# astojanov/Clover

Measured on AMD Instinct MI355X. Metric: int4 GEMV (CloverMatrix4::mvm) effective GB/s, algorithmic operand bytes / time, higher is better.
Workload: dtype int4; 1 GPU; CloverMatrix4::mvm 65536x65536 int4 (65536x65536 per GPU; preset c3: BASELINE configs[2] per GPU), x and result CloverVector4, STOCHASTIC_ROUNDING_DISABLED, bit-exact reference order; rows_per_gpu=65536, cols=65536, parallelism=row-shard x1, settle_launches=168

## Files before the change

clover_amd/csrc/matrix4.hip:

```cpp
#include "rng_device.h"

#include <stdlib.h>
#include <string.h>


#define MVM_CHUNK 65536u

template <int U, bool NT>
__device__ __forceinline__ void mvm_steps(const u32x4 *__restrict__ Ap, const u32x4 *xs, const float *cs, int q,
                                          uint32_t t0, float &a0, float &a1, float &a2, float &a3)
{
    u32x4 a[U];
#pragma unroll
    for (int u = 0; u < U; u++) a[u] = NT ? __builtin_nontemporal_load(&Ap[4 * (t0 + u) + q]) : Ap[4 * (t0 + u) + q];
#pragma unroll
    for (int u = 0; u < U; u++) {
        const u32x4 xv = xs[4 * (t0 + u) + q];
        const float c = cs[2 * (t0 + u) + (q >> 1)];
        a0 = __builtin_fmaf(c, (float)sdot8(a[u].x, xv.x, 0), a0);
        a1 = __builtin_fmaf(c, (float)sdot8(a[u].y, xv.y, 0), a1);
        a2 = __builtin_fmaf(c, (float)sdot8(a[u].z, xv.z, 0), a2);
        a3 = __builtin_fmaf(c, (float)sdot8(a[u].w, xv.w, 0), a3);
    }
}

template <int U, bool NT>
__device__ __forceinline__ void mvm_steps8(const u32x2 *__restrict__ Ap, const u32x2 *xs, const float *cs, int e, uint32_t t0, float &a0,
                                           float &a1)
{
    u32x2 a[U];
#pragma unroll
    for (int u = 0; u < U; u++) a[u] = NT ? __builtin_nontemporal_load(&Ap[8 * (t0 + u) + e]) : Ap[8 * (t0 + u) + e];
#pragma unroll
    for (int u = 0; u < U; u++) {
        const u32x2 xv = xs[8 * (t0 + u) + e];
        const float c = cs[2 * (t0 + u) + (e >> 2)];
        a0 = __builtin_fmaf(c, (float)sdot8(a[u].x, xv.x, 0), a0);
        a1 = __builtin_fmaf(c, (float)sdot8(a[u].y, xv.y, 0), a1);
    }
}

__device__ __forceinline__ int requantize_wave(float d, float noise, uint32_t *r_words, float *sr, float *scale)
{
    const int lane = threadIdx.x & 63;
    float m = wave_max(__builtin_fabsf(d));
    m = fix_zero_max(m);
    const float k = 7.0f / m;
    const int qv = quant1(d, k, noise);
    if (r_words) {
        uint32_t w = ((uint32_t)qv & 0xFu) << nib_shift(lane & 7);
        w |= __shfl_xor(w, 1);
        w |= __shfl_xor(w, 2);
        w |= __shfl_xor(w, 4);
        if ((lane & 7) == 0) r_words[lane >> 3] = w;
        if (lane == 0) *sr = m;
    }
    *scale = m;
    return qv;
}

struct MvmFuse {
    const uint32_t *qu;
    const float *su;
    float a;
    uint32_t *r2;
    float *sr2;
};

template <int U, bool NT, bool ST, bool FUSE, int L = 4>
__global__ __launch_bounds__(64 * L) void k_m4_mvm64(const uint8_t *__restrict__ A, const float *__restrict__ sA,
                                                  uint64_t cols, const uint8_t *__restrict__ x, const float *__restrict__ sx,
                                                  float *__restrict__ d_out, uint32_t *r, float *sr,
                                                  uint64_t *rng_state, uint64_t seq, const uint64_t *__restrict__ pow_rows, MvmFuse fuse)
{
    extern __shared__ __attribute__((aligned(16))) char smem[];
    u32x4 *xs = reinterpret_cast<u32x4 *>(smem);
    float *cs = reinterpret_cast<float *>(smem + MVM_CHUNK / 2);
    float *dsh = cs + MVM_CHUNK / 64;
    uint64_t *rbase = reinterpret_cast<uint64_t *>(dsh + 64);
    uint64_t *raw = rbase + 4;
    uint64_t *rbase2 = raw + 8, *raw2 = rbase2 + 4;
    if (ST) {
        const uint64_t a0 = rng_workgroup_begin(rng_state, seq, pow_rows, blockIdx.x, 1, (FUSE ? 4ull : 2ull) * gridDim.x, rbase);
        if (FUSE) {
            const uint64_t b2 = wave_pow_apply(pow_rows, a0, (uint64_t)gridDim.x + blockIdx.x, 1);
            if ((threadIdx.x & 63) == 0) rbase2[threadIdx.x >> 6] = b2;
        }
    }
    uint32_t fuse_w = 0;
    float fuse_s = 0.0f;
    if (FUSE && threadIdx.x < 64) {
        fuse_w = fuse.qu[blockIdx.x * 8 + (threadIdx.x >> 3)];
        fuse_s = fuse.su[blockIdx.x];
    }

    static_assert(L == 4 || (L == 8 && !ST), "the stochastic epilogue assumes 4 waves");
    constexpr int THREADS = 64 * L;
    const uint64_t rb = blockIdx.x;
    const int tid = threadIdx.x;
    const int q = tid & (L - 1);
    const int rho = tid / L;
    const uint64_t row = rb * 64 + rho;
    const u32x4 *Arow = reinterpret_cast<const u32x4 *>(A + row * (cols / 2));
    const float *sArow = sA + rb * (cols / 64);

    float a0 = 0.0f, a1 = 0.0f, a2 = 0.0f, a3 = 0.0f;

    for (uint64_t c0 = 0; c0 < cols; c0 += MVM_CHUNK) {
        const uint32_t cw = (uint32_t)((cols - c0) < MVM_CHUNK ? (cols - c0) : MVM_CHUNK);
        if (c0) __syncthreads();
        const u32x4 *xg = reinterpret_cast<const u32x4 *>(x + c0 / 2);
        {
            constexpr int NX = MVM_CHUNK / 32 / THREADS;
            constexpr int NC = MVM_CHUNK / 64 / THREADS;
            u32x4 xr[NX];
            float sa[NC], sv[NC];
            const uint32_t nx = cw / 32, nc = cw / 64;
#pragma unroll
            for (int k = 0; k < NX; k++) { const uint32_t i = tid + THREADS * k; xr[k] = xg[i < nx ? i : 0]; }
#pragma unroll
            for (int k = 0; k < NC; k++) {
                const uint32_t i = tid + THREADS * k, ii = i < nc ? i : 0;
                sa[k] = sArow[c0 / 64 + ii];
                sv[k] = sx[c0 / 64 + ii];
            }
#pragma unroll
            for (int k = 0; k < NX; k++) { const uint32_t i = tid + THREADS * k; if (i < nx) xs[i] = xr[k]; }
#pragma unroll
            for (int k = 0; k < NC; k++) { const uint32_t i = tid + THREADS * k; if (i < nc) cs[i] = (sa[k] * CLV_RCP49) * sv[k]; }
        }
        __syncthreads();

        const u32x4 *Ap = Arow + c0 / 32;
        const uint32_t npairs = cw / 128;
        uint32_t t = 0;
        if constexpr (L == 4) {
            for (; t + U <= npairs; t += U) mvm_steps<U, NT>(Ap, xs, cs, q, t, a0, a1, a2, a3);
            for (; t < npairs; t++) mvm_steps<1, NT>(Ap, xs, cs, q, t, a0, a1, a2, a3);
        } else {
            const u32x2 *Ap8 = reinterpret_cast<const u32x2 *>(Ap);
            const u32x2 *xs8 = reinterpret_cast<const u32x2 *>(xs);
            for (; t + U <= npairs; t += U) mvm_steps8<U, NT>(Ap8, xs8, cs, q, t, a0, a1);
            for (; t < npairs; t++) mvm_steps8<1, NT>(Ap8, xs8, cs, q, t, a0, a1);
        }
    }

    const float v0 = a0 + __shfl_xor(a0, 2);
    const float v1 = a1 + __shfl_xor(a1, 2);
    const float v2 = a2 + __shfl_xor(a2, 2);
    const float v3 = a3 + __shfl_xor(a3, 2);
    const float x0 = v0 + __shfl_xor(v0, 1);
    const float x1 = v1 + __shfl_xor(v1, 1);
    const float x2 = v2 + __shfl_xor(v2, 1);
    const float x3 = v3 + __shfl_xor(v3, 1);
    float dot = (x0 + x2) + (x1 + x3);
    if constexpr (L == 8) {
        const float u0 = a0 + __shfl_xor(a0, 4), u1 = a1 + __shfl_xor(a1, 4);
        const float y0 = u0 + __shfl_xor(u0, 2), y1 = u1 + __shfl_xor(u1, 2);
        const float z0 = y0 + __shfl_xor(y0, 1), z1 = y1 + __shfl_xor(y1, 1);
        dot = z0 + z1;
    }

    if (q == 0) {
        dsh[rho] = dot;
        if (d_out) d_out[row] = dot;
    }
    if (ST && tid < 4) {
        gen_blocks(rbase[tid], 1, raw, tid);
        if (FUSE) gen_blocks(rbase2[tid], 1, raw2, tid);
    }
    __syncthreads();
    if ((r || FUSE) && tid < 64) {
        float noise = 0.0f;
        if (ST) {
            const int grp = tid & 7, j = tid >> 3;
            noise = noise_of(reinterpret_cast<const uint32_t *>(raw + (size_t)(grp >> 2) * 4)[j], grp & 3);
        }
        float m;
        const int qv = requantize_wave(dsh[tid], noise, r ? r + rb * 8 : nullptr, r ? sr + rb : nullptr, &m);
        if (FUSE) {
            const float su7 = div7(fuse_s), sv7 = div7(m * fuse.a);
            const float val = __builtin_fmaf((float)qv, sv7, (float)unpack1(fuse_w, tid & 7) * su7);
            float noise2 = 0.0f;
            if (ST) {
                const int g = (tid & 7) ^ 1, j = tid >> 3;
                noise2 = noise_of(reinterpret_cast<const uint32_t *>(raw2 + (size_t)(g >> 2) * 4)[j], g & 3);
            }
            float m2;
            requantize_wave(val, noise2, fuse.r2 + rb * 8, fuse.sr2 + rb, &m2);
        }
    }
}

__global__ __launch_bounds__(256) void k_m4_quantize_strip(const float *__restrict__ A, uint64_t cols, uint32_t *__restrict__ q,
                                                           float *__restrict__ s, uint32_t strips_x, uint32_t tiles_x)
{
    __shared__ float sh[4][4];
    const uint32_t sj = blockIdx.x % strips_x;
    const uint64_t bi = blockIdx.x / strips_x;
    const int wave = threadIdx.x >> 6, lane = threadIdx.x & 63;
    const uint64_t col = (uint64_t)sj * 256 + 4 * lane;
    const bool live = col < cols;
    const uint64_t row0 = bi * 64 + wave * 16;

    f32x4 v[16];
    float m = 0.0f;
#pragma unroll
    for (int r = 0; r < 16; r++) {
        v[r] = live ? __builtin_nontemporal_load(reinterpret_cast<const f32x4 *>(A + (row0 + r) * cols + col)) : f32x4{0.0f, 0.0f, 0.0f, 0.0f};
        m = fmaxf(m, fmaxf(fmaxf(__builtin_fabsf(v[r].x), __builtin_fabsf(v[r].y)), fmaxf(__builtin_fabsf(v[r].z), __builtin_fabsf(v[r].w))));
    }
    m = row16_max(m);
    if ((lane & 15) == 0) sh[wave][lane >> 4] = m;
    __syncthreads();
    const int t = lane >> 4;
    m = fix_zero_max(fmaxf(fmaxf(sh[0][t], sh[1][t]), fmaxf(sh[2][t], sh[3][t])));
    const float k = 7.0f / m;
    if (wave == 0 && (lane & 15) == 0 && live) s[bi * tiles_x + sj * 4 + t] = m;
    const int odd = lane & 1;
#pragma unroll
    for (int r = 0; r < 16; r += 2) {
        const uint32_t h0 = quant_pack4(v[r], k), h1 = quant_pack4(v[r + 1], k);
        const uint32_t give = odd ? h0 : h1;
        const uint32_t recv = (uint32_t)__builtin_amdgcn_update_dpp(0, (int)give, 0xB1, 0xF, 0xF, false);
        const uint32_t word = odd ? (recv | (h1 << 16)) : (h0 | (recv << 16));
        if (live) __builtin_nontemporal_store(word, &q[((row0 + r + odd) * cols + (col & ~7ull)) / 8]);
    }
}

__global__ __launch_bounds__(256) void k_m4_gemm_simple(const uint8_t *__restrict__ A, const float *__restrict__ sA, uint64_t M,
                                                        uint64_t K, const uint8_t *__restrict__ B, const float *__restrict__ sB,
                                                        uint64_t N, float *__restrict__ C)
{
    const uint64_t j = (uint64_t)blockIdx.x * 16 + (threadIdx.x & 15);
    const uint64_t i = (uint64_t)blockIdx.y * 16 + (threadIdx.x >> 4);
    if (i >= M || j >= N) return;
    const uint64_t kb = K / 64;
    const u32x4 *a = reinterpret_cast<const u32x4 *>(A + i * (K / 2));
    const u32x4 *b = reinterpret_cast<const u32x4 *>(B + j * (K / 2));
    const float *sa = sA + (i >> 6) * kb;
    const float *sb = sB + (j >> 6) * kb;
    float acc = 0.0f;
    for (uint64_t blk = 0; blk < kb; blk++) {
        const int S = dot32(a[2 * blk], b[2 * blk]) + dot32(a[2 * blk + 1], b[2 * blk + 1]);
        const float c = (sa[blk] * CLV_RCP49) * sb[blk];
        acc = __builtin_fmaf(c, (float)S, acc);
    }
    C[i * N + j] = acc;
}

template <bool NT>
__global__ __launch_bounds__(256) void k_m4_restore(const uint32_t *__restrict__ q, const float *__restrict__ s, f32x4 *__restrict__ A,
                                                    uint64_t nquads, uint64_t cols)
{
    const uint64_t f0 = ((uint64_t)blockIdx.x * 4 + (threadIdx.x >> 6)) * 256;
    const int lane = threadIdx.x & 63;
    const uint64_t tiles_x = cols / 64;
    uint32_t wd[4];
    float sc[4];
#pragma unroll
    for (int j = 0; j < 4; j++) {
        const uint64_t f = f0 + 64 * j + lane, fc = f < nquads ? f : 0;
        const uint64_t e = fc * 4, row = e / cols, col = e - row * cols;
        wd[j] = q[fc >> 1];
        sc[j] = s[(row >> 6) * tiles_x + (col >> 6)];
    }
#pragma unroll
    for (int j = 0; j < 4; j++) {
        const uint64_t f = f0 + 64 * j + lane;
        const uint32_t hw = wd[j] >> (16 * (lane & 1));
        const float k = div7(sc[j]);
        f32x4 v;
        v.x = (float)(((int)(hw << 24)) >> 28) * k;
        v.y = (float)(((int)(hw << 28)) >> 28) * k;
        v.z = (float)(((int)(hw << 16)) >> 28) * k;
        v.w = (float)(((int)(hw << 20)) >> 28) * k;
        if (f < nquads) {
            if (NT) __builtin_nontemporal_store(v, &A[f]);
            else A[f] = v;
        }
    }
}

int clm4_quantize_stochastic(const float *A, uint64_t rows, uint64_t cols, int8_t *q, float *s, uint64_t *rng, hipStream_t st);
int clm4_gemm_mfma(const int8_t *A, const float *sA, uint64_t M, uint64_t K, const int8_t *B, const float *sB, uint64_t N, float *C, hipStream_t st);
int clm4_gemm_fp6(const int8_t *A, const float *sA, uint64_t M, uint64_t K, const int8_t *B, const float *sB, uint64_t N, float *C, hipStream_t st);

#define MVM_LDS_BYTES (MVM_CHUNK / 2 + (MVM_CHUNK / 64) * sizeof(float) + 64 * sizeof(float) + 256)

static int launch_mvm(const int8_t *A, const float *sA, uint64_t rows, uint64_t cols, const int8_t *x, const float *sx,
                      float *d, int8_t *r, float *sr, uint64_t *rng, hipStream_t st, const MvmFuse *fuse = nullptr)
{
    const size_t lds = MVM_LDS_BYTES;
    const dim3 grid((unsigned)(rows / 64)), block(256);
    RngTables T = {nullptr, nullptr, nullptr};
    uint64_t seq = 0;
    if (rng) {
        int rc = clv_rng_tables(&T);
        if (rc) return rc;
        seq = clv_rng_seq_for(rng, st);
    }
    const MvmFuse no_fuse = {nullptr, nullptr, 0.0f, nullptr, nullptr};
#define MVM_LAUNCH_F(NT, ST, FUSE)                                                                                               \
    hipLaunchKernelGGL((k_m4_mvm64<8, NT, ST, FUSE>), grid, block, lds, st, (const uint8_t *)A, sA, cols, (const uint8_t *)x, sx, d, \
                       (uint32_t *)r, sr, rng, seq, T.pow_rows, FUSE ? *fuse : no_fuse)
#define MVM_LAUNCH(NT, ST)                                  \
    do {                                                    \
        if (fuse) MVM_LAUNCH_F(NT, ST, true);               \
        else MVM_LAUNCH_F(NT, ST, false);                   \
    } while (0)
    const bool streaming = rows * (cols / 2) > (256ull << 20);
    const bool wide = streaming && !rng && rows / 64 <= 2ull * (uint64_t)clv_cu_count();
    if (wide) {
        if (fuse)
            hipLaunchKernelGGL((k_m4_mvm64<16, true, false, true, 8>), grid, dim3(512), lds, st, (const uint8_t *)A, sA, cols,
                               (const uint8_t *)x, sx, d, (uint32_t *)r, sr, rng, seq, T.pow_rows, *fuse);
        else
            hipLaunchKernelGGL((k_m4_mvm64<16, true, false, false, 8>), grid, dim3(512), lds, st, (const uint8_t *)A, sA, cols,
                               (const uint8_t *)x, sx, d, (uint32_t *)r, sr, rng, seq, T.pow_rows, no_fuse);
    } else if (streaming) {
        if (rng) MVM_LAUNCH(true, true); else MVM_LAUNCH(true, false);
    } else {
        if (rng) MVM_LAUNCH(false, true); else MVM_LAUNCH(false, false);
    }
#undef MVM_LAUNCH
#undef MVM_LAUNCH_F
    CLV_LAUNCH_CHECK();
    return CLV_OK;
}

#ifdef CLV_EXPERIMENTS
__global__ __launch_bounds__(256) void k_read_bw(const u32x4 *__restrict__ p, uint64_t n16, uint32_t *__restrict__ out, int nt)
{
    const uint64_t stride = (uint64_t)gridDim.x * blockDim.x;
    uint32_t acc = 0;
    uint64_t i = (uint64_t)blockIdx.x * blockDim.x + threadIdx.x;
    for (; i + 7 * stride < n16; i += 8 * stride) {
        u32x4 v[8];
#pragma unroll
        for (int u = 0; u < 8; u++) v[u] = nt ? __builtin_nontemporal_load(&p[i + u * stride]) : p[i + u * stride];
#pragma unroll
        for (int u = 0; u < 8; u++) acc ^= v[u].x ^ v[u].y ^ v[u].z ^ v[u].w;
    }
    for (; i < n16; i += stride) { const u32x4 v = p[i]; acc ^= v.x ^ v.y ^ v.z ^ v.w; }
    if (acc == 0x12345678u) out[0] = acc;
}

extern "C" int clvx_read_bw(const void *p, uint64_t bytes, int nt, int blocks_per_cu, void *out, void *stream)
{
    hipLaunchKernelGGL(k_read_bw, dim3(clv_cu_count() * blocks_per_cu), dim3(256), 0, as_stream(stream), (const u32x4 *)p, bytes / 16,
                       (uint32_t *)out, nt);
    CLV_LAUNCH_CHECK();
    return CLV_OK;
}

extern "C" int clvx_mvm_variant(int variant, const int8_t *A, const float *sA, uint64_t rows, uint64_t cols, const int8_t *x,
                                const float *sx, int8_t *r, float *sr, void *stream)
{
    const size_t lds = MVM_LDS_BYTES;
    hipStream_t st = as_stream(stream);
    const dim3 grid((unsigned)(rows / 64)), block(256);
#define CLVX_LAUNCH(U, NT)                                                                                                      \
    hipLaunchKernelGGL((k_m4_mvm64<U, NT, false, false>), grid, block, lds, st, (const uint8_t *)A, sA, cols, (const uint8_t *)x, sx, \
                       (float *)nullptr, (uint32_t *)r, sr, (uint64_t *)nullptr, 0ull, (const uint64_t *)nullptr,                      \
                       MvmFuse{nullptr, nullptr, 0.0f, nullptr, nullptr})
    switch (variant) {
    case 0: CLVX_LAUNCH(8, true); break;
    case 1: CLVX_LAUNCH(8, false); break;
    case 2: CLVX_LAUNCH(4, true); break;
    case 3: CLVX_LAUNCH(16, true); break;
    case 4: CLVX_LAUNCH(2, true); break;
    case 5: CLVX_LAUNCH(16, false); break;
    case 6: CLVX_LAUNCH(32, false); break;
#define CLVX_LAUNCH8(U, NT)                                                                                                       \
    hipLaunchKernelGGL((k_m4_mvm64<U, NT, false, false, 8>), grid, dim3(512), lds, st, (const uint8_t *)A, sA, cols, (const uint8_t *)x, \
                       sx, (float *)nullptr, (uint32_t *)r, sr, (uint64_t *)nullptr, 0ull, (const uint64_t *)nullptr,                 \
                       MvmFuse{nullptr, nullptr, 0.0f, nullptr, nullptr})
    case 7: CLVX_LAUNCH8(8, false); break;
    case 8: CLVX_LAUNCH8(16, false); break;
    case 9: CLVX_LAUNCH8(8, true); break;
    case 10: CLVX_LAUNCH8(16, true); break;
#undef CLVX_LAUNCH8
    default: clv_set_error("clvx_mvm_variant: unknown variant %d", variant); return CLV_ERR_INVALID;
    }
#undef CLVX_LAUNCH
    CLV_LAUNCH_CHECK();
    return CLV_OK;
}
#endif

static int check_mvm_args(const char *fn, const void *A, const void *sA, uint64_t rows, uint64_t cols, const void *x, const void *sx)
{
    CLV_REQUIRE(A && sA && x && sx, "%s: null pointer", fn);
    CLV_REQUIRE(rows % 64 == 0 && cols % 128 == 0, "%s: rows=%llu must be a multiple of 64 and cols=%llu of 128", fn,
                (unsigned long long)rows, (unsigned long long)cols);
    CLV_REQUIRE(rows / 64 <= 0x7FFFFFFFull, "%s: too many rows", fn);
    return CLV_OK;
}

extern "C" int clm4_restore(const int8_t *q, const float *s, uint64_t rows, uint64_t cols, float *A, void *stream)
{
    CLV_REQUIRE(A && q && s, "clm4_restore: null pointer");
    CLV_REQUIRE(rows % 128 == 0 && cols % 128 == 0, "clm4_restore: rows=%llu cols=%llu must be multiples of 128", (unsigned long long)rows,
                (unsigned long long)cols);
    if (!rows || !cols) return CLV_OK;
    const uint64_t nquads = rows * cols / 4, waves = (nquads + 255) / 256;
    CLV_REQUIRE((waves + 3) / 4 <= 0x7FFFFFFFull, "clm4_restore: matrix too large");
    if (rows * cols * sizeof(float) > (256ull << 20))
        hipLaunchKernelGGL(k_m4_restore<true>, dim3((unsigned)((waves + 3) / 4)), dim3(256), 0, as_stream(stream), (const uint32_t *)q, s,
                           (f32x4 *)A, nquads, cols);
    else
        hipLaunchKernelGGL(k_m4_restore<false>, dim3((unsigned)((waves + 3) / 4)), dim3(256), 0, as_stream(stream), (const uint32_t *)q, s,
                           (f32x4 *)A, nquads, cols);
    CLV_LAUNCH_CHECK();
    return CLV_OK;
}

extern "C" int clm4_mvm(const int8_t *A, const float *sA, uint64_t rows, uint64_t cols, const int8_t *x, const float *sx,
                        int8_t *r, float *sr, uint64_t *rng_state_dev, void *stream)
{
    int rc = check_mvm_args("clm4_mvm", A, sA, rows, cols, x, sx);
    if (rc) return rc;
    CLV_REQUIRE(r && sr, "clm4_mvm: null result pointer");
    if (!rows) return CLV_OK;
    hipStream_t st = as_stream(stream);
    return launch_mvm(A, sA, rows, cols, x, sx, nullptr, r, sr, rng_state_dev, st);
}

extern "C" int clm4_mvm_scale_and_add(const int8_t *A, const float *sA, uint64_t rows, uint64_t cols, const int8_t *x, const float *sx,
                                      const int8_t *qu, const float *su, float a, int8_t *t, float *st_, int8_t *r, float *sr,
                                      uint64_t *rng_state_dev, void *stream)
{
    int rc = check_mvm_args("clm4_mvm_scale_and_add", A, sA, rows, cols, x, sx);
    if (rc) return rc;
    CLV_REQUIRE(qu && su && r && sr, "clm4_mvm_scale_and_add: null pointer");
    CLV_REQUIRE((t == nullptr) == (st_ == nullptr), "clm4_mvm_scale_and_add: t and st must both be given or both be NULL");
    CLV_REQUIRE((const void *)r != (const void *)x && (const void *)sr != (const void *)sx,
                "clm4_mvm_scale_and_add: the result must not alias the vector being multiplied");
    if (!rows) return CLV_OK;
    const MvmFuse fuse = {(const uint32_t *)qu, su, a, (uint32_t *)r, sr};
    return launch_mvm(A, sA, rows, cols, x, sx, nullptr, t, st_, rng_state_dev, as_stream(stream), &fuse);
}

extern "C" int clm4_rowdots(const int8_t *A, const float *sA, uint64_t rows, uint64_t cols, const int8_t *x, const float *sx,
                            float *d, void *stream)
{
    int rc = check_mvm_args("clm4_rowdots", A, sA, rows, cols, x, sx);
    if (rc) return rc;
    CLV_REQUIRE(d, "clm4_rowdots: null result pointer");
    if (!rows) return CLV_OK;
    return launch_mvm(A, sA, rows, cols, x, sx, d, nullptr, nullptr, nullptr, as_stream(stream));
}

extern "C" int clm4_quantize(const float *A, uint64_t rows, uint64_t cols, int8_t *q, float *s, uint64_t *rng_state_dev, void *stream)
{
    CLV_REQUIRE(A && q && s, "clm4_quantize: null pointer");
    CLV_REQUIRE(rows % 128 == 0 && cols % 128 == 0, "clm4_quantize: rows=%llu cols=%llu must be multiples of 128",
                (unsigned long long)rows, (unsigned long long)cols);
    if (!rows || !cols) return CLV_OK;
    const uint64_t tiles = (rows / 64) * (cols / 64);
    CLV_REQUIRE(tiles <= 0x7FFFFFFFull, "clm4_quantize: too many tiles");
    if (rng_state_dev) return clm4_quantize_stochastic(A, rows, cols, q, s, rng_state_dev, as_stream(stream));
    const uint32_t strips_x = (uint32_t)((cols + 255) / 256);
    hipLaunchKernelGGL(k_m4_quantize_strip, dim3((unsigned)((rows / 64) * strips_x)), dim3(256), 0, as_stream(stream), A, cols,
                       (uint32_t *)q, s, strips_x, (uint32_t)(cols / 64));
    CLV_LAUNCH_CHECK();
    return CLV_OK;
}

extern "C" int clm4_gemm(const int8_t *A, const float *sA, uint64_t M, uint64_t K, const int8_t *B, const float *sB, uint64_t N,
                         float *C, void *stream)
{
    CLV_REQUIRE(A && sA && B && sB && C, "clm4_gemm: null pointer");
    CLV_REQUIRE(M % 128 == 0 && N % 128 == 0 && K % 128 == 0, "clm4_gemm: M=%llu N=%llu K=%llu must be multiples of 128",
                (unsigned long long)M, (unsigned long long)N, (unsigned long long)K);
    if (!M || !N) return CLV_OK;
    static const int which = [] { const char *e = clv_env("CLV_GEMM_KERNEL"); return !e ? 0 : !strcmp(e, "simple") ? 2 : !strcmp(e, "i8") ? 1 : 0; }();
    if (which == 0 && K > 0) return clm4_gemm_fp6(A, sA, M, K, B, sB, N, C, as_stream(stream));
    if (which == 1 && K > 0) return clm4_gemm_mfma(A, sA, M, K, B, sB, N, C, as_stream(stream));
    hipLaunchKernelGGL(k_m4_gemm_simple, dim3((unsigned)(N / 16), (unsigned)(M / 16)), dim3(256), 0, as_stream(stream),
                       (const uint8_t *)A, sA, M, K, (const uint8_t *)B, sB, N, C);
    CLV_LAUNCH_CHECK();
    return CLV_OK;
}
```

Baseline: 6542 GB/s.

## Stage x chunk via global_load_lds and prefetch first A tile before barrier

The x-vector staging into LDS now uses direct global-to-LDS loads instead of a register round trip, and the first U matrix tiles are issued before the __syncthreads so their latency overlaps the x/scale staging. Timestamp probes (compiled only under CLV_PROBE) are added to measure per-block phases. The cost removed is the serialized prologue where A loads waited for the x staging barrier. It adds register pressure from holding U tiles across the barrier, and the experiment launch paths pass g_mvm_stamps unconditionally, which looks inconsistent if CLV_PROBE is off.

```diff
diff --git a/clover_amd/csrc/matrix4.hip b/clover_amd/csrc/matrix4.hip
--- a/clover_amd/csrc/matrix4.hip
+++ b/clover_amd/csrc/matrix4.hip
@@ -2,17 +2,23 @@
 
 #include <stdlib.h>
 #include <string.h>
+#include <type_traits>
 
 
 #define MVM_CHUNK 65536u
 
-template <int U, bool NT>
-__device__ __forceinline__ void mvm_steps(const u32x4 *__restrict__ Ap, const u32x4 *xs, const float *cs, int q,
-                                          uint32_t t0, float &a0, float &a1, float &a2, float &a3)
-{
-    u32x4 a[U];
-#pragma unroll
-    for (int u = 0; u < U; u++) a[u] = NT ? __builtin_nontemporal_load(&Ap[4 * (t0 + u) + q]) : Ap[4 * (t0 + u) + q];
+template <int U, bool NT, typename V>
+__device__ __forceinline__ void mvm_load(const V *__restrict__ Ap, int q, uint32_t t0, V (&a)[U])
+{
+    constexpr int LN = 64 / sizeof(V);
+#pragma unroll
+    for (int u = 0; u < U; u++) a[u] = NT ? __builtin_nontemporal_load(&Ap[LN * (t0 + u) + q]) : Ap[LN * (t0 + u) + q];
+}
+
+template <int U>
+__device__ __forceinline__ void mvm_consume(const u32x4 (&a)[U], const u32x4 *xs, const float *cs, int q, uint32_t t0, float &a0,
+                                            float &a1, float &a2, float &a3)
+{
 #pragma unroll
     for (int u = 0; u < U; u++) {
         const u32x4 xv = xs[4 * (t0 + u) + q];
@@ -24,13 +30,10 @@
     }
 }
 
-template <int U, bool NT>
-__device__ __forceinline__ void mvm_steps8(const u32x2 *__restrict__ Ap, const u32x2 *xs, const float *cs, int e, uint32_t t0, float &a0,
-                                           float &a1)
-{
-    u32x2 a[U];
-#pragma unroll
-    for (int u = 0; u < U; u++) a[u] = NT ? __builtin_nontemporal_load(&Ap[8 * (t0 + u) + e]) : Ap[8 * (t0 + u) + e];
+template <int U>
+__device__ __forceinline__ void mvm_consume8(const u32x2 (&a)[U], const u32x2 *xs, const float *cs, int e, uint32_t t0, float &a0,
+                                             float &a1)
+{
 #pragma unroll
     for (int u = 0; u < U; u++) {
         const u32x2 xv = xs[8 * (t0 + u) + e];
@@ -38,6 +41,24 @@
         a0 = __builtin_fmaf(c, (float)sdot8(a[u].x, xv.x, 0), a0);
         a1 = __builtin_fmaf(c, (float)sdot8(a[u].y, xv.y, 0), a1);
     }
+}
+
+template <int U, bool NT>
+__device__ __forceinline__ void mvm_steps(const u32x4 *__restrict__ Ap, const u32x4 *xs, const float *cs, int q,
+                                          uint32_t t0, float &a0, float &a1, float &a2, float &a3)
+{
+    u32x4 a[U];
+    mvm_load<U, NT>(Ap, q, t0, a);
+    mvm_consume<U>(a, xs, cs, q, t0, a0, a1, a2, a3);
+}
+
+template <int U, bool NT>
+__device__ __forceinline__ void mvm_steps8(const u32x2 *__restrict__ Ap, const u32x2 *xs, const float *cs, int e, uint32_t t0, float &a0,
+                                           float &a1)
+{
+    u32x2 a[U];
+    mvm_load<U, NT>(Ap, e, t0, a);
+    mvm_consume8<U>(a, xs, cs, e, t0, a0, a1);
 }
 
 __device__ __forceinline__ int requantize_wave(float d, float noise, uint32_t *r_words, float *sr, float *scale)
@@ -67,11 +88,17 @@
     float *sr2;
 };
 
+#define MVM_STAMP(k) CLV_PROBE(do { if (dbg && threadIdx.x == 0) dbg[(size_t)blockIdx.x * 8 + (k)] = __builtin_amdgcn_s_memrealtime(); } while (0))
+
+typedef __attribute__((address_space(1))) const void m4_gptr_t;
+typedef __attribute__((address_space(3))) void m4_lptr_t;
+
 template <int U, bool NT, bool ST, bool FUSE, int L = 4>
 __global__ __launch_bounds__(64 * L) void k_m4_mvm64(const uint8_t *__restrict__ A, const float *__restrict__ sA,
                                                   uint64_t cols, const uint8_t *__restrict__ x, const float *__restrict__ sx,
                                                   float *__restrict__ d_out, uint32_t *r, float *sr,
-                                                  uint64_t *rng_state, uint64_t seq, const uint64_t *__restrict__ pow_rows, MvmFuse fuse)
+                                                  uint64_t *rng_state, uint64_t seq, const uint64_t *__restrict__ pow_rows, MvmFuse fuse
+                                                  CLV_PROBE(, unsigned long long *dbg))
 {
     extern __shared__ __attribute__((aligned(16))) char smem[];
     u32x4 *xs = reinterpret_cast<u32x4 *>(smem);
@@ -106,18 +133,24 @@
 
     float a0 = 0.0f, a1 = 0.0f, a2 = 0.0f, a3 = 0.0f;
 
+    using AV = typename std::conditional<L == 4, u32x4, u32x2>::type;
+    const int wave = __builtin_amdgcn_readfirstlane(tid >> 6), lane = tid & 63;
+
+    MVM_STAMP(0);
     for (uint64_t c0 = 0; c0 < cols; c0 += MVM_CHUNK) {
         const uint32_t cw = (uint32_t)((cols - c0) < MVM_CHUNK ? (cols - c0) : MVM_CHUNK);
         if (c0) __syncthreads();
         const u32x4 *xg = reinterpret_cast<const u32x4 *>(x + c0 / 2);
+        const AV *Ap = reinterpret_cast<const AV *>(Arow + c0 / 32);
+        const AV *xv = reinterpret_cast<const AV *>(xs);
+        const uint32_t npairs = cw / 128;
+        const bool ahead = npairs >= (uint32_t)U;
+        AV a[U];
         {
-            constexpr int NX = MVM_CHUNK / 32 / THREADS;
+            constexpr int NP = MVM_CHUNK / 32 / THREADS;
             constexpr int NC = MVM_CHUNK / 64 / THREADS;
-            u32x4 xr[NX];
             float sa[NC], sv[NC];
             const uint32_t nx = cw / 32, nc = cw / 64;
-#pragma unroll
-            for (int k = 0; k < NX; k++) { const uint32_t i = tid + THREADS * k; xr[k] = xg[i < nx ? i : 0]; }
 #pragma unroll
             for (int k = 0; k < NC; k++) {
                 const uint32_t i = tid + THREADS * k, ii = i < nc ? i : 0;
@@ -125,25 +158,31 @@
                 sv[k] = sx[c0 / 64 + ii];
             }
 #pragma unroll
-            for (int k = 0; k < NX; k++) { const uint32_t i = tid + THREADS * k; if (i < nx) xs[i] = xr[k]; }
+            for (int k = 0; k < NP; k++) {
+                const uint32_t p = wave + (THREADS / 64) * k, i = 64 * p + lane;
+                if (i < nx) __builtin_amdgcn_global_load_lds((m4_gptr_t *)(xg + i), (m4_lptr_t *)(smem + 1024 * p), 16, 0, 0);
+            }
+            if (ahead) mvm_load<U, NT>(Ap, q, 0, a);
 #pragma unroll
             for (int k = 0; k < NC; k++) { const uint32_t i = tid + THREADS * k; if (i < nc) cs[i] = (sa[k] * CLV_RCP49) * sv[k]; }
         }
         __syncthreads();
-
-        const u32x4 *Ap = Arow + c0 / 32;
-        const uint32_t npairs = cw / 128;
+        MVM_STAMP(1);
+
         uint32_t t = 0;
         if constexpr (L == 4) {
-            for (; t + U <= npairs; t += U) mvm_steps<U, NT>(Ap, xs, cs, q, t, a0, a1, a2, a3);
-            for (; t < npairs; t++) mvm_steps<1, NT>(Ap, xs, cs, q, t, a0, a1, a2, a3);
+            if (ahead) { mvm_consume<U>(a, xv, cs, q, 0, a0, a1, a2, a3); t = U; }
+            MVM_STAMP(2);
+            for (; t + U <= npairs; t += U) mvm_steps<U, NT>(Ap, xv, cs, q, t, a0, a1, a2, a3);
+            for (; t < npairs; t++) mvm_steps<1, NT>(Ap, xv, cs, q, t, a0, a1, a2, a3);
         } else {
-            const u32x2 *Ap8 = reinterpret_cast<const u32x2 *>(Ap);
-            const u32x2 *xs8 = reinterpret_cast<const u32x2 *>(xs);
-            for (; t + U <= npairs; t += U) mvm_steps8<U, NT>(Ap8, xs8, cs, q, t, a0, a1);
-            for (; t < npairs; t++) mvm_steps8<1, NT>(Ap8, xs8, cs, q, t, a0, a1);
+            if (ahead) { mvm_consume8<U>(a, xv, cs, q, 0, a0, a1); t = U; }
+            MVM_STAMP(2);
+            for (; t + U <= npairs; t += U) mvm_steps8<U, NT>(Ap, xv, cs, q, t, a0, a1);
+            for (; t < npairs; t++) mvm_steps8<1, NT>(Ap, xv, cs, q, t, a0, a1);
         }
     }
+    MVM_STAMP(3);
 
     const float v0 = a0 + __shfl_xor(a0, 2);
     const float v1 = a1 + __shfl_xor(a1, 2);
@@ -190,6 +229,7 @@
             requantize_wave(val, noise2, fuse.r2 + rb * 8, fuse.sr2 + rb, &m2);
         }
     }
+    MVM_STAMP(4);
 }
 
 __global__ __launch_bounds__(256) void k_m4_quantize_strip(const float *__restrict__ A, uint64_t cols, uint32_t *__restrict__ q,
@@ -286,6 +326,8 @@
 int clm4_gemm_mfma(const int8_t *A, const float *sA, uint64_t M, uint64_t K, const int8_t *B, const float *sB, uint64_t N, float *C, hipStream_t st);
 int clm4_gemm_fp6(const int8_t *A, const float *sA, uint64_t M, uint64_t K, const int8_t *B, const float *sB, uint64_t N, float *C, hipStream_t st);
 
+CLV_PROBE(static unsigned long long *g_mvm_stamps = nullptr;)
+
 #define MVM_LDS_BYTES (MVM_CHUNK / 2 + (MVM_CHUNK / 64) * sizeof(float) + 64 * sizeof(float) + 256)
 
 static int launch_mvm(const int8_t *A, const float *sA, uint64_t rows, uint64_t cols, const int8_t *x, const float *sx,
@@ -303,7 +345,7 @@
     const MvmFuse no_fuse = {nullptr, nullptr, 0.0f, nullptr, nullptr};
 #define MVM_LAUNCH_F(NT, ST, FUSE)                                                                                               \
     hipLaunchKernelGGL((k_m4_mvm64<8, NT, ST, FUSE>), grid, block, lds, st, (const uint8_t *)A, sA, cols, (const uint8_t *)x, sx, d, \
-                       (uint32_t *)r, sr, rng, seq, T.pow_rows, FUSE ? *fuse : no_fuse)
+                       (uint32_t *)r, sr, rng, seq, T.pow_rows, FUSE ? *fuse : no_fuse CLV_PROBE(, g_mvm_stamps))
 #define MVM_LAUNCH(NT, ST)                                  \
     do {                                                    \
         if (fuse) MVM_LAUNCH_F(NT, ST, true);               \
@@ -314,10 +356,10 @@
     if (wide) {
         if (fuse)
             hipLaunchKernelGGL((k_m4_mvm64<16, true, false, true, 8>), grid, dim3(512), lds, st, (const uint8_t *)A, sA, cols,
-                               (const uint8_t *)x, sx, d, (uint32_t *)r, sr, rng, seq, T.pow_rows, *fuse);
+                               (const uint8_t *)x, sx, d, (uint32_t *)r, sr, rng, seq, T.pow_rows, *fuse CLV_PROBE(, g_mvm_stamps));
         else
             hipLaunchKernelGGL((k_m4_mvm64<16, true, false, false, 8>), grid, dim3(512), lds, st, (const uint8_t *)A, sA, cols,
-                               (const uint8_t *)x, sx, d, (uint32_t *)r, sr, rng, seq, T.pow_rows, no_fuse);
+                               (const uint8_t *)x, sx, d, (uint32_t *)r, sr, rng, seq, T.pow_rows, no_fuse CLV_PROBE(, g_mvm_stamps));
     } else if (streaming) {
         if (rng) MVM_LAUNCH(true, true); else MVM_LAUNCH(true, false);
     } else {
@@ -351,6 +393,12 @@
     hipLaunchKernelGGL(k_read_bw, dim3(clv_cu_count() * blocks_per_cu), dim3(256), 0, as_stream(stream), (const u32x4 *)p, bytes / 16,
                        (uint32_t *)out, nt);
     CLV_LAUNCH_CHECK();
+    return CLV_OK;
+}
+
+extern "C" int clvx_mvm_stamps(void *buf)
+{
+    g_mvm_stamps = (unsigned long long *)buf;
     return CLV_OK;
 }
 
@@ -363,7 +411,7 @@
 #define CLVX_LAUNCH(U, NT)                                                                                                      \
     hipLaunchKernelGGL((k_m4_mvm64<U, NT, false, false>), grid, block, lds, st, (const uint8_t *)A, sA, cols, (const uint8_t *)x, sx, \
                        (float *)nullptr, (uint32_t *)r, sr, (uint64_t *)nullptr, 0ull, (const uint64_t *)nullptr,                      \
-                       MvmFuse{nullptr, nullptr, 0.0f, nullptr, nullptr})
+                       MvmFuse{nullptr, nullptr, 0.0f, nullptr, nullptr}, g_mvm_stamps)
     switch (variant) {
     case 0: CLVX_LAUNCH(8, true); break;
     case 1: CLVX_LAUNCH(8, false); break;
@@ -375,7 +423,7 @@
 #define CLVX_LAUNCH8(U, NT)                                                                                                       \
     hipLaunchKernelGGL((k_m4_mvm64<U, NT, false, false, 8>), grid, dim3(512), lds, st, (const uint8_t *)A, sA, cols, (const uint8_t *)x, \
                        sx, (float *)nullptr, (uint32_t *)r, sr, (uint64_t *)nullptr, 0ull, (const uint64_t *)nullptr,                 \
-                       MvmFuse{nullptr, nullptr, 0.0f, nullptr, nullptr})
+                       MvmFuse{nullptr, nullptr, 0.0f, nullptr, nullptr}, g_mvm_stamps)
     case 7: CLVX_LAUNCH8(8, false); break;
     case 8: CLVX_LAUNCH8(16, false); break;
     case 9: CLVX_LAUNCH8(8, true); break;
```

After: 6430 GB/s. 1.7% lower.
